# ZongyueQin/SessionSimilaritySearch

Hardware: AMD Instinct MI355X
Metric: session queries/sec (higher is better)
Workload: dtype f32

## Files before the change

sessionsimilaritysearch_amd/csrc/scan_dev.h:

```cpp
#pragma once
#include "scan.h"

namespace sss {

typedef char __attribute__((address_space(3)))* lptr_c;
typedef __bf16 bf16x8 __attribute__((ext_vector_type(8)));
typedef _Float16 f16x8 __attribute__((ext_vector_type(8)));
typedef int i32x4 __attribute__((ext_vector_type(4)));
typedef int i32x16 __attribute__((ext_vector_type(16)));

template <int N>
__device__ __forceinline__ void list_insert(float (&ls)[N], int (&li)[N], float x, int id) {
#pragma unroll
    for (int i = 0; i < N; ++i) {
        const bool c = x > ls[i];
        const float ns = c ? x : ls[i];
        const int ni = c ? id : li[i];
        x = c ? ls[i] : x;
        id = c ? li[i] : id;
        ls[i] = ns;
        li[i] = ni;
    }
}

__device__ __forceinline__ float vmax3(float a, float b, float c) {
    float r;
    asm("v_max3_f32 %0, %1, %2, %3" : "=v"(r) : "v"(a), "v"(b), "v"(c));
    return r;
}

__device__ __forceinline__ unsigned min8_sc1(const unsigned* p) {
    u32x4 a, b;
    asm volatile("global_load_dwordx4 %0, %2, off sc1\n\t"
                 "global_load_dwordx4 %1, %2, off offset:16 sc1\n\t"
                 "s_waitcnt vmcnt(0)"
                 : "=&v"(a), "=&v"(b) : "v"(p) : "memory");
    const unsigned m0 = min(min(a.x, a.y), min(a.z, a.w));
    const unsigned m1 = min(min(b.x, b.y), min(b.z, b.w));
    return min(m0, m1);
}

__device__ __forceinline__ void cx_u32(unsigned& a, unsigned& b) {
    const unsigned lo = min(a, b), hi = max(a, b);
    a = lo; b = hi;
}

__device__ __forceinline__ unsigned tau_select16(unsigned (&v)[8], int skip, int h) {
    cx_u32(v[0], v[1]); cx_u32(v[2], v[3]); cx_u32(v[4], v[5]); cx_u32(v[6], v[7]);
    cx_u32(v[0], v[2]); cx_u32(v[1], v[3]); cx_u32(v[4], v[6]); cx_u32(v[5], v[7]);
    cx_u32(v[1], v[2]); cx_u32(v[5], v[6]); cx_u32(v[0], v[4]); cx_u32(v[3], v[7]);
    cx_u32(v[1], v[5]); cx_u32(v[2], v[6]);
    cx_u32(v[1], v[4]); cx_u32(v[3], v[6]);
    cx_u32(v[2], v[4]); cx_u32(v[3], v[5]);
    cx_u32(v[3], v[4]);
    const int m = (skip >> 1) + ((skip & 1) && h == 0 ? 1 : 0);
    unsigned mine = v[0];
    mine = m >= 1 ? v[1] : mine;
    mine = m >= 2 ? v[2] : mine;
    mine = m >= 3 ? v[3] : mine;
    mine = m >= 4 ? v[4] : mine;
    return min(mine, (unsigned)__shfl_xor((int)mine, 32));
}

__device__ __forceinline__ void load8_sc1(const unsigned* p, unsigned (&v)[8]) {
    u32x4 a, b;
    asm volatile("global_load_dwordx4 %0, %2, off sc1\n\t"
                 "global_load_dwordx4 %1, %2, off offset:16 sc1\n\t"
                 "s_waitcnt vmcnt(0)"
                 : "=&v"(a), "=&v"(b) : "v"(p) : "memory");
    v[0] = a.x; v[1] = a.y; v[2] = a.z; v[3] = a.w; v[4] = b.x; v[5] = b.y; v[6] = b.z; v[7] = b.w;
}

template <int RB, int DT>
__device__ __forceinline__ void load_queries(const char* __restrict__ Qb, int q_ld, int h, f32x4 (&qc)[RB / 32], int* q_shift = nullptr) {
    constexpr int NU = RB / 32;
    if constexpr (DT == DT_SPLIT) {
        const f32x4* qp = reinterpret_cast<const f32x4*>(Qb + (size_t)q_ld * RB) + 2 * h;
#pragma unroll
        for (int u = 0; u < NU / 2; ++u) {
            const f32x4 a = qp[4 * u], b = qp[4 * u + 1];
            const float x[8] = {a.x, a.y, a.z, a.w, b.x, b.y, b.z, b.w};
            bf16x8 hi, lo;
#pragma unroll
            for (int e = 0; e < 8; ++e) {
                hi[e] = (__bf16)x[e];
                const float rem = x[e] - (float)hi[e];
                lo[e] = (__bf16)(__builtin_isfinite(rem) ? rem : 0.f);
            }
            qc[u] = __builtin_bit_cast(f32x4, hi);
            qc[u + NU / 2] = __builtin_bit_cast(f32x4, lo);
        }
#pragma unroll
        for (int u = 0; u < NU; ++u) asm volatile("" : "+v"(qc[u]));
    } else if constexpr (DT == DT_F16) {
        const f32x4* qp = reinterpret_cast<const f32x4*>(Qb + (size_t)q_ld * (2 * RB)) + 2 * h;
        f32x4 raw[2 * NU];
        float amax = 0.f;
#pragma unroll
        for (int u = 0; u < NU; ++u) { raw[2 * u] = qp[4 * u]; raw[2 * u + 1] = qp[4 * u + 1]; }
#pragma unroll
        for (int u = 0; u < 2 * NU; ++u)
            amax = fmaxf(fmaxf(amax, fmaxf(fabsf(raw[u].x), fabsf(raw[u].y))), fmaxf(fabsf(raw[u].z), fabsf(raw[u].w)));
        amax = fmaxf(amax, __shfl_xor(amax, 32));
        const int sh = f16_shift(amax);
        if (q_shift) *q_shift = sh;
#pragma unroll
        for (int u = 0; u < NU; ++u) {
            const f32x4 a = raw[2 * u], b = raw[2 * u + 1];
            f16x8 v;
            v[0] = (_Float16)ldexpf(a.x, sh); v[1] = (_Float16)ldexpf(a.y, sh);
            v[2] = (_Float16)ldexpf(a.z, sh); v[3] = (_Float16)ldexpf(a.w, sh);
            v[4] = (_Float16)ldexpf(b.x, sh); v[5] = (_Float16)ldexpf(b.y, sh);
            v[6] = (_Float16)ldexpf(b.z, sh); v[7] = (_Float16)ldexpf(b.w, sh);
            qc[u] = __builtin_bit_cast(f32x4, v);
        }
#pragma unroll
        for (int u = 0; u < NU; ++u) asm volatile("" : "+v"(qc[u]));
    } else {
        const f32x4* qp = reinterpret_cast<const f32x4*>(Qb + (size_t)q_ld * RB) + h;
#pragma unroll
        for (int u = 0; u < NU; ++u) qc[u] = qp[2 * u];
#pragma unroll
        for (int u = 0; u < NU; ++u) asm volatile("" : "+v"(qc[u]));
    }

}

}
```

sessionsimilaritysearch_amd/csrc/scan_kernel.h:

```cpp
#pragma once
#include "scan.h"
#include "scan_dev.h"

#ifndef SSS_STAGGER
#define SSS_STAGGER 1
#endif

namespace sss {

extern __device__ unsigned g_boot_expired;

template <int RB, int TR, int DT, int NW, bool THR = false, bool AP = false, int MET = 0>
__global__ __launch_bounds__(NW * 64, AP ? 2 * (NW / 4) : NW / 4) void k_scan(const ScanArgs A) {
    constexpr int H = TR / 64;
    constexpr int CH = RB / 16;
    constexpr int NU = RB / 32;
    constexpr int TILE_BYTES = TR * RB;
    constexpr int LOADS_PER_WAVE = TR * CH / 64 / NW;
    constexpr int WGQ = NW * 32;
    constexpr bool PRECOMP = RB <= 512 && !AP;
    constexpr int TAU_LDS = 2 * TILE_BYTES;
    static_assert(CH <= 64, "row longer than one LDS-DMA instruction");
    static_assert(LOADS_PER_WAVE >= 1, "a tile is at least one DMA piece per wave");
    extern __shared__ __attribute__((aligned(16))) char smem[];

    const int nq = A.nq, n = A.n, S = A.S, G = A.G, J = A.J;
    const char* __restrict__ Qb = reinterpret_cast<const char*>(A.Q);
    const char* __restrict__ Cb = reinterpret_cast<const char*>(A.C);
    const int tid = threadIdx.x;
    const int lane = tid & 63;
    const int wave = __builtin_amdgcn_readfirstlane(tid >> 6);
    const int r = lane & 31, h = lane >> 5;

    const int bid = blockIdx.x;
    const int xcd = bid & 7, slot = bid >> 3;
    const int split = xcd * (S >> 3) + slot / G;
    const int g = slot % G;

    const int q_local = wave * 32 + r;
    const int q_glob = g * WGQ + q_local;
    int q_ld = q_glob < nq ? q_glob : nq - 1;
    if constexpr (THR) q_ld = A.qsel[q_ld];
    f32x4 qc[NU];

    float ls[KP];
    int li[KP];
#pragma unroll
    for (int i = 0; i < KP; ++i) { ls[i] = -INFINITY; li[i] = -1; }
    float pend_s = -INFINITY;
    int pend_i = -1;
    constexpr int E = 4;
    float es[E];
    int ei[E];
    int ecnt = 0;
#pragma unroll
    for (int i = 0; i < E; ++i) { es[i] = -INFINITY; ei[i] = -1; }
    float tau = -INFINITY, thr = -INFINITY;
    if constexpr (THR) thr = q_glob < nq ? A.thr[q_glob] : INFINITY;
    float rmax = -INFINITY;
    float pub = -INFINITY;

    int tile_lo = split * A.tiles_per_split;
    int tile_hi = tile_lo + A.tiles_per_split;
    if (tile_hi > A.total_tiles) tile_hi = A.total_tiles;
    const int ntiles = tile_lo < tile_hi ? tile_hi - tile_lo : 0;
    const bool use_tau = !THR && J > 0;
    const bool boot = use_tau && A.boot && ntiles > 0;
    const int nb = boot ? 1 : 0;
    const int niter = ntiles + nb;
    auto tile_of = [&](int i) { return i < ntiles ? tile_lo + i : tile_lo; };
    const int skip = A.tau_skip;

    bool slots_seen = false;
    const unsigned* my_half = nullptr;
    unsigned cls_live = 0;
#ifdef SSS_EXP_NOPAIR
    const bool pair_pub = false;
#else
    const bool pair_pub = A.cert == 1;
#endif
    if (use_tau) {
        cls_live = pair_pub ? (unsigned)(split + (split >> 4)) & 15u : (unsigned)(2 * split + h) % (unsigned)A.Ju;
        my_half = A.slots + (size_t)q_ld * SLOT_STRIDE + h * (J >> 1);
    }
    auto tau_ord = [&]() -> unsigned {
        if (J == 16 && skip > 0) {
            unsigned v[8];
            load8_sc1(my_half, v);
            return tau_select16(v, skip, h);
        }
        unsigned m = 0xFFFFFFFFu;
        for (int v = 0; v < (J >> 1); v += 8) m = min(m, min8_sc1(my_half + v));
        return min(m, (unsigned)__shfl_xor((int)m, 32));
    };
    const unsigned tau_lds = (unsigned)(unsigned long)(lptr_c)smem + TAU_LDS + wave * 2048;
    auto tau_fetch = [&]() {
        int ln = lane;
        asm volatile("" : "+v"(ln));
#pragma unroll
        for (int j = 0; j < 2; ++j) {
            int qi = g * WGQ + wave * 32 + 16 * j + (ln >> 2);
            if (qi > nq - 1) qi = nq - 1;
            const unsigned off = (unsigned)qi * (unsigned)(SLOT_STRIDE * 4) + (unsigned)(ln & 3) * 16u;
            const unsigned dst = __builtin_amdgcn_readfirstlane(tau_lds + j * 1024);
            asm volatile("s_mov_b32 m0, %1\n\ts_nop 0\n\tglobal_load_lds_dwordx4 %0, %2 sc1"
                         : : "v"(off), "s"(dst), "s"(A.slots) : "memory");
        }
    };
    auto tau_read = [&]() -> unsigned {
        const u32x4* p = reinterpret_cast<const u32x4*>(smem + TAU_LDS + wave * 2048 + r * 64 + h * 32);
        const u32x4 a = p[0], b = p[1];
        if (skip > 0) {
            unsigned v[8] = {a.x, a.y, a.z, a.w, b.x, b.y, b.z, b.w};
            return tau_select16(v, skip, h);
        }
        const unsigned m = min(min(min(a.x, a.y), min(a.z, a.w)), min(min(b.x, b.y), min(b.z, b.w)));
        return min(m, (unsigned)__shfl_xor((int)m, 32));
    };
    auto set_tau = [&](unsigned m) {
        if (m > ORD_NEG_INF) tau = fmaxf(tau, ord2f(m - 1));
        thr = AP ? tau : fmaxf(ls[KP - 1], tau);
    };
    auto publish = [&](unsigned cls) {
        float val = rmax;
        bool ok = true;
        if (A.cert > 1) {
            float v2 = ls[1], v4 = ls[3], v8 = ls[7], v16 = ls[KP - 1];
            int i2 = li[1], i4 = li[3], i8 = li[7], i16 = li[KP - 1];
            asm volatile("" : "+v"(v2), "+v"(v4), "+v"(v8), "+v"(v16), "+v"(i2), "+v"(i4), "+v"(i8), "+v"(i16));
            const int c = A.cert;
            val = c == 2 ? v2 : c == 4 ? v4 : c == 8 ? v8 : v16;
            ok = (c == 2 ? i2 : c == 4 ? i4 : c == 8 ? i8 : i16) >= 0;
        }
        if (pair_pub) { val = fmaxf(val, __shfl_xor(val, 32)); ok = h == 0; }
        unsigned cur = 0u;
        if (J == 16 && slots_seen) cur = *reinterpret_cast<const unsigned*>(smem + TAU_LDS + wave * 2048 + r * 64 + cls * 4u);
        if (ok && val > pub && val > tau && f2ord(val) > cur && q_glob < nq) {
            int qq = THR ? q_ld : q_glob;
            asm volatile("" : "+v"(qq));
            __hip_atomic_fetch_max(A.slots + ((size_t)(unsigned)qq * (unsigned)SLOT_STRIDE + cls), f2ord(val), __ATOMIC_RELAXED, __HIP_MEMORY_SCOPE_AGENT);
            pub = val;
        }
    };

    const unsigned lds_base = (unsigned)(unsigned long)(lptr_c)smem;
    auto slot_row = [&](int i) { return ((wave * LOADS_PER_WAVE + i) * 64 + lane) / CH; };
    auto slot_off = [&](int i) {
        const int p = (wave * LOADS_PER_WAVE + i) * 64 + lane;
        const int tr = p / CH, sc = p % CH;
        return (unsigned)(tr * RB + ((sc ^ (tr & 15)) * 16));
    };
    unsigned lane_off[PRECOMP ? LOADS_PER_WAVE : 1];
    if (PRECOMP) {
#pragma unroll
        for (int i = 0; i < LOADS_PER_WAVE; ++i) lane_off[i] = slot_off(i);
    }
    auto stage_piece = [&](int buf, int tile_idx, int i) {
        const long row0 = (long)tile_idx * TR;
        const bool inside = row0 + TR <= (long)n;
        const char* tile_src = Cb + (size_t)row0 * RB;
        const unsigned dst = __builtin_amdgcn_readfirstlane(
            lds_base + buf * TILE_BYTES + (wave * LOADS_PER_WAVE + i) * 1024);
        unsigned off = PRECOMP ? lane_off[PRECOMP ? i : 0] : slot_off(i);
        if (!inside) {
            const int lr = slot_row(i);
            long grow = row0 + lr;
            if (grow > (long)n - 1) grow = (long)n - 1;
            off = (unsigned)((grow - row0) * RB) + (off - (unsigned)(lr * RB));
        }
        asm volatile("s_mov_b32 m0, %1\n\ts_nop 0\n\tglobal_load_lds_dwordx4 %0, %2"
                     : : "v"(off), "s"(dst), "s"(tile_src) : "memory");
    };
    auto stage = [&](int buf, int tile_idx) {
#pragma unroll
        for (int i = 0; i < LOADS_PER_WAVE; ++i) stage_piece(buf, tile_idx, i);
    };

    const int x = h ^ (r & 15);
    f32x16 acc0 = {0}, acc1 = {0};
    [[maybe_unused]] float bcur[MET ? 2 * H : 1];
    [[maybe_unused]] float bscale = 1.f;
    [[maybe_unused]] auto bias_fetch = [&](int tile_idx) {
#pragma unroll
        for (int s = 0; s < 2 * H; ++s) {
            long row = (long)tile_idx * TR + s * 32 + r;
            if (row > (long)n - 1) row = (long)n - 1;
            bcur[s] = h == 0 ? A.bias[row] : 0.f;
        }
    };
    [[maybe_unused]] auto bias_land = [&]() {
#pragma unroll
        for (int s = 0; s < 2 * H; ++s) asm volatile("" : "+v"(bcur[s]));
    };

    auto mfma_sub = [&](int buf, int sub, int next_tile) {
        const char* tile = smem + buf * TILE_BYTES + sub * (64 * RB);
        if constexpr (H == 1) { if (next_tile >= 0) stage(buf ^ 1, next_tile); }
        auto lda = [&](int u) -> const f32x4* {
            const int c = (2 * u) ^ x;
            return reinterpret_cast<const f32x4*>(tile + (r * CH + c) * 16);
        };
        constexpr int PF = DT == DT_F32 ? 1 : AP ? 1 : (RB == 256 ? NU : RB == 512 ? 4 : 2);
        f32x4 as0[NU], as1[NU];
#pragma unroll
        for (int u = 0; u < PF && u < NU; ++u) { const f32x4* p = lda(u); as0[u] = p[0]; as1[u] = p[32 * CH]; }
        const f32x16 zero = {0};
        if constexpr (MET) {
            float b0 = bcur[0], b1 = bcur[1];
#pragma unroll
            for (int s = 1; s < H; ++s) { b0 = sub == s ? bcur[2 * s] : b0; b1 = sub == s ? bcur[2 * s + 1] : b1; }
            acc0 = __builtin_amdgcn_mfma_f32_32x32x2f32(b0, bscale, zero, 0, 0, 0);
            acc1 = __builtin_amdgcn_mfma_f32_32x32x2f32(b1, bscale, zero, 0, 0, 0);
        } else {
            acc0 = zero; acc1 = zero;
        }
        [[maybe_unused]] i32x16 ia0 = {0}, ia1 = {0};
#pragma unroll
        for (int u = 0; u < NU; ++u) {
            if (u + PF < NU) { const f32x4* p = lda(u + PF); as0[u + PF] = p[0]; as1[u + PF] = p[32 * CH]; }
            const f32x4 a0 = as0[u], a1 = as1[u];
            __builtin_amdgcn_sched_barrier(0);
            if constexpr (DT == DT_F32) {
                acc0 = __builtin_amdgcn_mfma_f32_32x32x2f32(a0.x, qc[u].x, acc0, 0, 0, 0);
                acc1 = __builtin_amdgcn_mfma_f32_32x32x2f32(a1.x, qc[u].x, acc1, 0, 0, 0);
                acc0 = __builtin_amdgcn_mfma_f32_32x32x2f32(a0.y, qc[u].y, acc0, 0, 0, 0);
                acc1 = __builtin_amdgcn_mfma_f32_32x32x2f32(a1.y, qc[u].y, acc1, 0, 0, 0);
                acc0 = __builtin_amdgcn_mfma_f32_32x32x2f32(a0.z, qc[u].z, acc0, 0, 0, 0);
                acc1 = __builtin_amdgcn_mfma_f32_32x32x2f32(a1.z, qc[u].z, acc1, 0, 0, 0);
                acc0 = __builtin_amdgcn_mfma_f32_32x32x2f32(a0.w, qc[u].w, acc0, 0, 0, 0);
                acc1 = __builtin_amdgcn_mfma_f32_32x32x2f32(a1.w, qc[u].w, acc1, 0, 0, 0);
            } else if constexpr (DT == DT_BF16) {
                const bf16x8 qb = __builtin_bit_cast(bf16x8, qc[u]);
                acc0 = __builtin_amdgcn_mfma_f32_32x32x16_bf16(__builtin_bit_cast(bf16x8, a0), qb, acc0, 0, 0, 0);
                acc1 = __builtin_amdgcn_mfma_f32_32x32x16_bf16(__builtin_bit_cast(bf16x8, a1), qb, acc1, 0, 0, 0);
            } else if constexpr (DT == DT_F16 || DT == DT_H16) {
                const f16x8 qb = __builtin_bit_cast(f16x8, qc[u]);
                acc0 = __builtin_amdgcn_mfma_f32_32x32x16_f16(__builtin_bit_cast(f16x8, a0), qb, acc0, 0, 0, 0);
                acc1 = __builtin_amdgcn_mfma_f32_32x32x16_f16(__builtin_bit_cast(f16x8, a1), qb, acc1, 0, 0, 0);
            } else if constexpr (DT == DT_I8) {
                const i32x4 qb = __builtin_bit_cast(i32x4, qc[u]);
                ia0 = __builtin_amdgcn_mfma_i32_32x32x32_i8(__builtin_bit_cast(i32x4, a0), qb, ia0, 0, 0, 0);
                ia1 = __builtin_amdgcn_mfma_i32_32x32x32_i8(__builtin_bit_cast(i32x4, a1), qb, ia1, 0, 0, 0);
            } else {
                const bf16x8 A0 = __builtin_bit_cast(bf16x8, a0), A1 = __builtin_bit_cast(bf16x8, a1);
                const bf16x8 qh = __builtin_bit_cast(bf16x8, qc[u < NU / 2 ? u : u - NU / 2]);
                acc0 = __builtin_amdgcn_mfma_f32_32x32x16_bf16(A0, qh, acc0, 0, 0, 0);
                acc1 = __builtin_amdgcn_mfma_f32_32x32x16_bf16(A1, qh, acc1, 0, 0, 0);
                if (u < NU / 2) {
                    const bf16x8 ql = __builtin_bit_cast(bf16x8, qc[u + NU / 2]);
                    acc0 = __builtin_amdgcn_mfma_f32_32x32x16_bf16(A0, ql, acc0, 0, 0, 0);
                    acc1 = __builtin_amdgcn_mfma_f32_32x32x16_bf16(A1, ql, acc1, 0, 0, 0);
                }
            }
            __builtin_amdgcn_sched_barrier(0);
        }
        if constexpr (DT == DT_I8) {
            acc0 = __builtin_convertvector(ia0, f32x16);
            acc1 = __builtin_convertvector(ia1, f32x16);
        }
        if constexpr (H > 1) { if (sub == 0 && next_tile >= 0) stage(buf ^ 1, next_tile); }
    };

    auto block_max = [&](const f32x16& a, float& q0, float& q1, float& q2, float& q3) {
        q0 = fmaxf(fmaxf(a[0], a[1]), fmaxf(a[2], a[3]));
        q1 = fmaxf(fmaxf(a[4], a[5]), fmaxf(a[6], a[7]));
        q2 = fmaxf(fmaxf(a[8], a[9]), fmaxf(a[10], a[11]));
        q3 = fmaxf(fmaxf(a[12], a[13]), fmaxf(a[14], a[15]));
        return fmaxf(fmaxf(q0, q1), fmaxf(q2, q3));
    };
    auto insert_block = [&](const f32x16& a, int base) {
        float q0, q1, q2, q3;
        const float m = block_max(a, q0, q1, q2, q3);
        if (__builtin_amdgcn_ballot_w64(m > thr) == 0) return;
        auto walk = [&](float qm, int j0) {
            if (__builtin_amdgcn_ballot_w64(qm > thr) == 0) return;
#pragma unroll
            for (int jj = 0; jj < 4; ++jj) {
                const int j = j0 + jj;
                const bool pass = a[j] > thr;
                if (__builtin_amdgcn_ballot_w64(pass) != 0) {
                    if (__builtin_amdgcn_ballot_w64(pass && pend_i >= 0) != 0) {
                        list_insert<KP>(ls, li, pend_s, pend_i);
                        pend_s = -INFINITY; pend_i = -1;
                        thr = fmaxf(ls[KP - 1], tau);
                    }
                    const bool still = a[j] > thr;
                    pend_s = still ? a[j] : pend_s;
                    pend_i = still ? base + (j & 3) + 8 * (j >> 2) : pend_i;
                }
            }
        };
        walk(q0, 0); walk(q1, 4); walk(q2, 8); walk(q3, 12);
    };
    auto flush = [&](bool need) {
        if (need && q_glob < nq) {
            const unsigned at = atomicAdd(A.cnt + q_glob, (unsigned)ecnt);
            unsigned long long* dst = A.cand + (size_t)q_glob * A.cap;
            unsigned long long lost = 0ull;
#pragma unroll
            for (int i = 0; i < E; ++i) {
                if (i < ecnt) {
                    const unsigned long long key = make_key(es[i], ei[i]);
                    if (at + (unsigned)i < (unsigned)A.cap) dst[at + i] = key;
                    else lost = lost > key ? lost : key;
                }
            }
            if (lost != 0ull && A.maxlast != nullptr) atomicMax(A.maxlast + q_glob, lost);
        }
        ecnt = need ? 0 : ecnt;
    };
    auto append_block = [&](const f32x16& a, int base) {
        float q0, q1, q2, q3;
        const float m = block_max(a, q0, q1, q2, q3);
        if (__builtin_amdgcn_ballot_w64(m > thr) == 0) return;
        auto walk = [&](float qm, int j0) {
            if (__builtin_amdgcn_ballot_w64(qm > thr) == 0) return;
#pragma unroll
            for (int jj = 0; jj < 4; ++jj) {
                const int j = j0 + jj;
                const bool pass = a[j] > thr;
                if (__builtin_amdgcn_ballot_w64(pass) != 0) {
                    const bool full = pass && ecnt == E;
                    if (__builtin_amdgcn_ballot_w64(full) != 0) flush(full);
#pragma unroll
                    for (int i = E - 1; i > 0; --i) { es[i] = pass ? es[i - 1] : es[i]; ei[i] = pass ? ei[i - 1] : ei[i]; }
                    es[0] = pass ? a[j] : es[0];
                    ei[0] = pass ? base + (j & 3) + 8 * (j >> 2) : ei[0];
                    ecnt += pass ? 1 : 0;
                }
            }
        };
        walk(q0, 0); walk(q1, 4); walk(q2, 8); walk(q3, 12);
    };
    auto emit_block = [&](const f32x16& a, int base) {
        float q0, q1, q2, q3;
        const float m = block_max(a, q0, q1, q2, q3);
        if (__builtin_amdgcn_ballot_w64(m > thr) == 0) return;
#pragma unroll
        for (int j = 0; j < 16; ++j) {
            if (a[j] > thr) {
                const unsigned pos = atomicAdd(A.cnt + q_glob, 1u);
                if (pos < (unsigned)A.cap) A.cand[(size_t)q_glob * A.cap + pos] = make_key(a[j], base + (j & 3) + 8 * (j >> 2));
            }
        }
    };
    const bool two_ahead = H > 1 && niter > 1;
    if (ntiles > 0) stage(0, tile_lo);
    if (two_ahead) stage(1, tile_of(1));
    if constexpr (MET) {
        int q_shift = 0;
        load_queries<RB, DT>(Qb, q_ld, h, qc, &q_shift);
        if constexpr (DT == DT_F16) {
            const int e = A.corpus_shift + q_shift;
            bscale = ldexpf(1.f, e < -126 ? -126 : e > 127 ? 127 : e);
        }
        bias_fetch(tile_of(0));
    } else {
        load_queries<RB, DT>(Qb, q_ld, h, qc);
    }
    asm volatile("s_waitcnt vmcnt(0)" ::: "memory");
    __syncthreads();
    if constexpr (MET) bias_land();

    const int T = niter * H;
    long row0_of_step = 0;
    constexpr bool TAU_EVERY_TILE = TR >= 512;
    auto refresh_at = [&](int i) {
        if (i == 1 && boot && !TAU_EVERY_TILE) return false;
        if (TAU_EVERY_TILE || i <= 4) return true;
        const int sh = 30 - __builtin_clz(i);
        return (i & ((1 << sh) - 1)) == 0;
    };
    auto tile_top = [&](int i) {
        if (!use_tau || i == 0) return;
        if (J == 16) {
            if (!refresh_at(i)) return;
            publish(cls_live);
            tau_fetch();
            return;
        }
        const int ii = i - (wave >= 4 ? 1 : 0);
        if (ii >= 2 && (ii <= 8 || (ii & (ii - 1)) == 0 || (ii & 15) == 0)) set_tau(tau_ord());
        publish(cls_live);
    };
    auto tile_end = [&](int i) {
        const bool pre = boot && i == 0;
        if (pre) publish(cls_live);
        if constexpr (MET) { if (i + 1 < niter) bias_fetch(tile_of(i + 1)); }
        asm volatile("s_waitcnt vmcnt(0)" ::: "memory");
        if (use_tau && J == 16 && i > 0 && refresh_at(i)) { set_tau(tau_read()); slots_seen = true; }
        __syncthreads();
        if (pre) {
            unsigned m = 0;
            for (int it = 0; it < (AP ? 1024 : 24); ++it) {
                m = tau_ord();
                if (__builtin_amdgcn_ballot_w64(m == 0) == 0) break;
                __builtin_amdgcn_s_sleep(16);
            }
            if constexpr (!MET) {
                if (lane == 0 && __builtin_amdgcn_ballot_w64(m == 0 && q_glob < nq) != 0) atomicAdd(&g_boot_expired, 1u);
            }
            set_tau(m);
        }
        if constexpr (MET) bias_land();
    };
    auto score_mfma = [&](int t) {
        const int i = (int)((unsigned)t / (unsigned)H), sub = (int)((unsigned)t % (unsigned)H);
        if (sub == 0) tile_top(i);
        const int next_tile = (i + 1 < niter && !(two_ahead && i == 0)) ? tile_of(i + 1) : -1;
        mfma_sub(i & 1, sub, next_tile);
        row0_of_step = (long)tile_of(i) * TR + sub * 64;
        if (row0_of_step + 64 > n) {
#pragma unroll
            for (int j = 0; j < 16; ++j) {
                const int rr = (int)row0_of_step + 4 * h + (j & 3) + 8 * (j >> 2);
                if (rr >= n) acc0[j] = -INFINITY;
                if (rr + 32 >= n) acc1[j] = -INFINITY;
            }
        }
    };
    auto score_tree = [&]() -> float {
        float m0 = vmax3(acc0[0], acc0[1], acc0[2]), m1 = vmax3(acc1[0], acc1[1], acc1[2]);
#pragma unroll
        for (int j = 3; j < 15; j += 2) { m0 = vmax3(m0, acc0[j], acc0[j + 1]); m1 = vmax3(m1, acc1[j], acc1[j + 1]); }
        const float m = vmax3(m0, m1, acc0[15]);
        const float mm = vmax3(m, acc1[15], rmax);
        rmax = mm;
        return vmax3(m, acc1[15], acc1[15]);
    };
    const int t_live = nb * H;
    const bool defer = SSS_STAGGER && NW == 8 && (DT == DT_SPLIT || DT == DT_BF16 || DT == DT_H16 || DT == DT_I8) && wave >= 4;
    int t = 0;
    if constexpr (AP || THR) {
        t = T;
        for (int i = 0; i < niter; ++i) {
            tile_top(i);
            const int tile = tile_of(i);
            const int next_tile = (i + 1 < niter && !(two_ahead && i == 0)) ? tile_of(i + 1) : -1;
            const int row_base = tile * TR;
            const bool ragged = row_base + TR > n;
            const bool live = i >= nb;
            if constexpr (THR) {
                if (g * WGQ + wave * 32 >= nq) {
                    if (next_tile >= 0) stage((i & 1) ^ 1, next_tile);
                    tile_end(i);
                    continue;
                }
            }
#pragma unroll
            for (int sub = 0; sub < H; ++sub) {
                mfma_sub(i & 1, sub, next_tile);
                const int row0 = row_base + sub * 64;
                if (ragged) {
#pragma unroll
                    for (int j = 0; j < 16; ++j) {
                        const int rr = row0 + 4 * h + (j & 3) + 8 * (j >> 2);
                        if (rr >= n) acc0[j] = -INFINITY;
                        if (rr + 32 >= n) acc1[j] = -INFINITY;
                    }
                }
                const float m = score_tree();
                if (live && __builtin_amdgcn_ballot_w64(m > thr) != 0) {
                    append_block(acc0, row0 + 4 * h);
                    append_block(acc1, row0 + 32 + 4 * h);
                }
            }
            tile_end(i);
        }
    }
    while (t < T) {
        bool rare = false;
        for (; t < T; ++t) {
            const bool last = (unsigned)t % (unsigned)H == H - 1;
            const bool early = defer && t >= t_live;
            score_mfma(t);
            if (early && last) tile_end((int)((unsigned)t / (unsigned)H));
            const float m = score_tree();
            if (t >= t_live && __builtin_amdgcn_ballot_w64(m > thr) != 0) { rare = true; break; }
            if (!early && last) tile_end((int)((unsigned)t / (unsigned)H));
        }
        if (!rare) break;
        if constexpr (THR) {
            emit_block(acc0, (int)row0_of_step + 4 * h);
            emit_block(acc1, (int)row0_of_step + 32 + 4 * h);
        } else if constexpr (AP) {
            append_block(acc0, (int)row0_of_step + 4 * h);
            append_block(acc1, (int)row0_of_step + 32 + 4 * h);
        } else {
            insert_block(acc0, (int)row0_of_step + 4 * h);
            insert_block(acc1, (int)row0_of_step + 32 + 4 * h);
        }
        if (!defer && (unsigned)t % (unsigned)H == H - 1) tile_end((int)((unsigned)t / (unsigned)H));
        ++t;
    }
    if constexpr (THR) { flush(ecnt > 0); return; }
    if constexpr (AP) flush(ecnt > 0);
    list_insert<KP>(ls, li, pend_s, pend_i);
    if (!AP && q_glob < nq) {
        int nreal = 0;
#pragma unroll
        for (int i = 0; i < KP; ++i) nreal += li[i] >= 0 ? 1 : 0;
        if (nreal > 0) {
            const unsigned base = atomicAdd(A.cnt + q_glob, (unsigned)nreal);
            unsigned long long* dst = A.cand + (size_t)q_glob * A.cap + base;
#pragma unroll
            for (int i = 0; i < KP; ++i)
                if (i < nreal) dst[i] = make_key(ls[i], li[i]);
            if (nreal == KP) atomicMax(A.maxlast + q_glob, (unsigned long long)make_key(ls[KP - 1], li[KP - 1]));
        }
    }
}

template <int RB, int TR, int DT, int NW, int MET, bool THR, bool AP = false>
static int launch_form(const ScanArgs& a, hipStream_t st) {
    const size_t lds = 2 * (size_t)TR * RB + NW * 2048;
    const int rc = opt_in_lds(reinterpret_cast<const void*>(&k_scan<RB, TR, DT, NW, THR, AP, MET>), "k_scan", lds);
    if (rc) return rc;
    hipLaunchKernelGGL((k_scan<RB, TR, DT, NW, THR, AP, MET>), dim3(a.S * a.G), dim3(NW * 64), lds, st, a);
    return check_launch("k_scan");
}
template <int RB, int TR, int DT, int NW, int MET>
static int launch_one(const ScanArgs& a, hipStream_t st) {
    if (a.thr != nullptr) {
        if constexpr (TR == (RB <= 512 ? 128 : 64)) return launch_form<RB, TR, DT, NW, MET, true>(a, st);
        set_error("scan: threshold form not built for %d-row tiles of %d-byte rows", TR, RB);
        return SSS_EINVAL;
    }
    if (a.append) {
        if constexpr (RB == 256 && TR == 128 && DT != DT_F32) return launch_form<RB, TR, DT, NW, MET, false, true>(a, st);
        set_error("scan: append form not built for this shape");
        return SSS_EINVAL;
    }
    return launch_form<RB, TR, DT, NW, MET, false>(a, st);
}
template <int DT, int MET>
static int launch_shape(int rb, int tile_rows, const ScanArgs& a, hipStream_t st) {
    if (rb == 256) return tile_rows == 256 ? launch_one<256, 256, DT, 8, MET>(a, st) : launch_one<256, 128, DT, 8, MET>(a, st);
    if (rb == 512) return tile_rows == 128 ? launch_one<512, 128, DT, 8, MET>(a, st) : launch_one<512, 64, DT, 8, MET>(a, st);
    if (rb == 1024) return launch_one<1024, 64, DT, 4, MET>(a, st);
    return 1;
}

}
```

Baseline: 489,400.

## Add hand-scheduled f32 MFMA scan loop with spread DMA and early score tree

Adds a specialised main loop for the f32, RB=512, non-append path that software-pipelines LDS fragment reads one k-group ahead of the MFMAs. It fences the MFMA groups with sched_barrier, interleaves the next tile's LDS-DMA loads between k-groups, and starts the max-reduction on acc0 while acc1's last MFMAs are still in flight. The goal is to hide LDS latency, DMA issue cost and the score-tree tail behind matrix work. It adds considerable code complexity, a fixed s_nop delay before the first acc1 max, and brittle timing assumptions tied to compile-time flags.

After: 498,700, median of 6. 1.02x the previous value.

```diff
diff --git a/sessionsimilaritysearch_amd/csrc/scan_dev.h b/sessionsimilaritysearch_amd/csrc/scan_dev.h
--- a/sessionsimilaritysearch_amd/csrc/scan_dev.h
+++ b/sessionsimilaritysearch_amd/csrc/scan_dev.h
@@ -26,6 +26,12 @@
 __device__ __forceinline__ float vmax3(float a, float b, float c) {
     float r;
     asm("v_max3_f32 %0, %1, %2, %3" : "=v"(r) : "v"(a), "v"(b), "v"(c));
+    return r;
+}
+
+__device__ __forceinline__ float vmax3_settled(float a, float b, float c) {
+    float r;
+    asm volatile("s_nop 15\n\ts_nop 2\n\tv_max3_f32 %0, %1, %2, %3" : "=v"(r) : "v"(a), "v"(b), "v"(c));
     return r;
 }
 
diff --git a/sessionsimilaritysearch_amd/csrc/scan_kernel.h b/sessionsimilaritysearch_amd/csrc/scan_kernel.h
--- a/sessionsimilaritysearch_amd/csrc/scan_kernel.h
+++ b/sessionsimilaritysearch_amd/csrc/scan_kernel.h
@@ -4,6 +4,9 @@
 
 #ifndef SSS_STAGGER
 #define SSS_STAGGER 1
+#endif
+#ifndef SSS_F32_SCHED
+#define SSS_F32_SCHED 7
 #endif
 
 namespace sss {
@@ -20,6 +23,7 @@
     constexpr int WGQ = NW * 32;
     constexpr bool PRECOMP = RB <= 512 && !AP;
     constexpr int TAU_LDS = 2 * TILE_BYTES;
+    constexpr bool F32S = (SSS_F32_SCHED & 1) && DT == DT_F32 && !AP && !THR && RB == 512;
     static_assert(CH <= 64, "row longer than one LDS-DMA instruction");
     static_assert(LOADS_PER_WAVE >= 1, "a tile is at least one DMA piece per wave");
     extern __shared__ __attribute__((aligned(16))) char smem[];
@@ -468,7 +472,138 @@
             tile_end(i);
         }
     }
-    while (t < T) {
+    if constexpr (F32S) {
+        constexpr bool SPREAD = (SSS_F32_SCHED & 2) != 0, EARLY_TREE = (SSS_F32_SCHED & 4) != 0;
+        static_assert(LOADS_PER_WAVE + 1 < NU, "a DMA piece per k-group, behind k-groups 1 .. LOADS_PER_WAVE");
+        const unsigned frag_lane = (unsigned)(r * CH) * 16u;
+        f32x4 nf0 = {0}, nf1 = {0};
+        auto frag_ptr = [&](unsigned step_off, int u) -> const f32x4* {
+            const int c = (2 * u) ^ x;
+            return reinterpret_cast<const f32x4*>(smem + step_off + frag_lane + c * 16);
+        };
+        auto read_first = [&](unsigned step_off) { const f32x4* p = frag_ptr(step_off, 0); nf0 = p[0]; nf1 = p[32 * CH]; };
+        float tm0 = -INFINITY;
+        auto step = [&](int t) -> float {
+            const int i = (int)((unsigned)t / (unsigned)H), sub = (int)((unsigned)t % (unsigned)H);
+            const unsigned off = (unsigned)((i & 1) * TILE_BYTES + sub * (64 * RB));
+            f32x4 as0[NU], as1[NU];
+            as0[0] = nf0; as1[0] = nf1;
+            const f32x16 zero = {0};
+            if constexpr (MET) {
+                float b0 = bcur[0], b1 = bcur[1];
+#pragma unroll
+                for (int s = 1; s < H; ++s) { b0 = sub == s ? bcur[2 * s] : b0; b1 = sub == s ? bcur[2 * s + 1] : b1; }
+                acc0 = __builtin_amdgcn_mfma_f32_32x32x2f32(b0, bscale, zero, 0, 0, 0);
+                acc1 = __builtin_amdgcn_mfma_f32_32x32x2f32(b1, bscale, zero, 0, 0, 0);
+            } else {
+                acc0 = zero; acc1 = zero;
+            }
+            auto fetch = [&](int u) { const f32x4* p = frag_ptr(off, u); as0[u] = p[0]; as1[u] = p[32 * CH]; };
+            auto mfma8 = [&](int u) {
+                const f32x4 a0 = as0[u], a1 = as1[u];
+                __builtin_amdgcn_sched_barrier(0);
+                acc0 = __builtin_amdgcn_mfma_f32_32x32x2f32(a0.x, qc[u].x, acc0, 0, 0, 0);
+                acc1 = __builtin_amdgcn_mfma_f32_32x32x2f32(a1.x, qc[u].x, acc1, 0, 0, 0);
+                acc0 = __builtin_amdgcn_mfma_f32_32x32x2f32(a0.y, qc[u].y, acc0, 0, 0, 0);
+                acc1 = __builtin_amdgcn_mfma_f32_32x32x2f32(a1.y, qc[u].y, acc1, 0, 0, 0);
+                acc0 = __builtin_amdgcn_mfma_f32_32x32x2f32(a0.z, qc[u].z, acc0, 0, 0, 0);
+                acc1 = __builtin_amdgcn_mfma_f32_32x32x2f32(a1.z, qc[u].z, acc1, 0, 0, 0);
+                acc0 = __builtin_amdgcn_mfma_f32_32x32x2f32(a0.w, qc[u].w, acc0, 0, 0, 0);
+                acc1 = __builtin_amdgcn_mfma_f32_32x32x2f32(a1.w, qc[u].w, acc1, 0, 0, 0);
+                __builtin_amdgcn_sched_barrier(0);
+            };
+            fetch(1);
+            mfma8(0);
+            if (sub == 0) tile_top(i);
+            const int next_tile = (sub == 0 && i + 1 < niter && !(two_ahead && i == 0)) ? tile_of(i + 1) : -1;
+            const long nrow0 = (long)next_tile * TR;
+            const bool dma_plain = next_tile >= 0 && nrow0 + TR <= (long)n;
+            const char* dma_src = Cb + (size_t)nrow0 * RB;
+            const unsigned dma_dst = __builtin_amdgcn_readfirstlane(lds_base + ((i & 1) ^ 1) * TILE_BYTES + wave * LOADS_PER_WAVE * 1024);
+            row0_of_step = (long)tile_of(i) * TR + sub * 64;
+            const bool ragged_step = row0_of_step + 64 > n;
+            const bool ends_tile = sub == H - 1 && !(boot && i == 0);
+            if (next_tile >= 0 && (!dma_plain || !SPREAD)) stage((i & 1) ^ 1, next_tile);
+#pragma unroll
+            for (int u = 1; u < NU - 1; ++u) {
+                fetch(u + 1);
+                mfma8(u);
+                if constexpr (SPREAD) {
+                    if (u <= LOADS_PER_WAVE && dma_plain)
+                        asm volatile("s_mov_b32 m0, %1\n\ts_nop 0\n\tglobal_load_lds_dwordx4 %0, %2"
+                                     : : "v"(lane_off[u - 1]), "s"(dma_dst + (u - 1) * 1024), "s"(dma_src) : "memory");
+                }
+            }
+            constexpr int u = NU - 1;
+            if (ends_tile) {
+                asm volatile("" : "+v"(as0[u]), "+v"(as1[u]));
+                tile_end(i);
+            }
+            if (t + 1 < T && (sub < H - 1 || ends_tile))
+                read_first(sub == H - 1 ? (unsigned)(((i + 1) & 1) * TILE_BYTES) : off + 64 * RB);
+            if constexpr (!EARLY_TREE) {
+                mfma8(u);
+            } else {
+                const f32x4 a0 = as0[u], a1 = as1[u];
+                __builtin_amdgcn_sched_barrier(0);
+                acc0 = __builtin_amdgcn_mfma_f32_32x32x2f32(a0.x, qc[u].x, acc0, 0, 0, 0);
+                acc0 = __builtin_amdgcn_mfma_f32_32x32x2f32(a0.y, qc[u].y, acc0, 0, 0, 0);
+                acc0 = __builtin_amdgcn_mfma_f32_32x32x2f32(a0.z, qc[u].z, acc0, 0, 0, 0);
+                acc0 = __builtin_amdgcn_mfma_f32_32x32x2f32(a0.w, qc[u].w, acc0, 0, 0, 0);
+                __builtin_amdgcn_sched_barrier(0);
+                acc1 = __builtin_amdgcn_mfma_f32_32x32x2f32(a1.x, qc[u].x, acc1, 0, 0, 0);
+                acc1 = __builtin_amdgcn_mfma_f32_32x32x2f32(a1.y, qc[u].y, acc1, 0, 0, 0);
+                __builtin_amdgcn_sched_barrier(0);
+                if (ragged_step) {
+#pragma unroll
+                    for (int j = 0; j < 16; ++j)
+                        if ((int)row0_of_step + 4 * h + (j & 3) + 8 * (j >> 2) >= n) acc0[j] = -INFINITY;
+                }
+                tm0 = vmax3(acc0[0], acc0[1], acc0[2]);
+#pragma unroll
+                for (int j = 3; j < 15; j += 2) tm0 = vmax3(tm0, acc0[j], acc0[j + 1]);
+                __builtin_amdgcn_sched_barrier(0);
+                acc1 = __builtin_amdgcn_mfma_f32_32x32x2f32(a1.z, qc[u].z, acc1, 0, 0, 0);
+                acc1 = __builtin_amdgcn_mfma_f32_32x32x2f32(a1.w, qc[u].w, acc1, 0, 0, 0);
+                __builtin_amdgcn_sched_barrier(0);
+            }
+            if (ragged_step) {
+#pragma unroll
+                for (int j = 0; j < 16; ++j) {
+                    const int rr = (int)row0_of_step + 4 * h + (j & 3) + 8 * (j >> 2);
+                    if (!EARLY_TREE && rr >= n) acc0[j] = -INFINITY;
+                    if (rr + 32 >= n) acc1[j] = -INFINITY;
+                }
+            }
+            if constexpr (!EARLY_TREE) return score_tree();
+            float m1 = vmax3_settled(acc1[0], acc1[1], acc1[2]);
+#pragma unroll
+            for (int j = 3; j < 15; j += 2) m1 = vmax3(m1, acc1[j], acc1[j + 1]);
+            const float m = vmax3(tm0, m1, acc0[15]);
+            rmax = vmax3(m, acc1[15], rmax);
+            return vmax3(m, acc1[15], acc1[15]);
+        };
+        if (T > 0) read_first(0);
+        while (t < T) {
+            bool rare = false;
+            for (; t < T; ++t) {
+                const float m = step(t);
+                if (t < t_live) {
+                    if (t == t_live - 1) {
+                        tile_end(0);
+                        if (t + 1 < T) read_first((unsigned)TILE_BYTES);
+                    }
+                    continue;
+                }
+                if (__builtin_amdgcn_ballot_w64(m > thr) != 0) { rare = true; break; }
+            }
+            if (!rare) break;
+            insert_block(acc0, (int)row0_of_step + 4 * h);
+            insert_block(acc1, (int)row0_of_step + 32 + 4 * h);
+            ++t;
+        }
+    }
+    while (!F32S && t < T) {
         bool rare = false;
         for (; t < T; ++t) {
             const bool last = (unsigned)t % (unsigned)H == H - 1;
```
